# Sunshine-718/AlphaZero-AL

Hardware: AMD Instinct MI355X
Metric: self-play positions/sec (Connect4 n_playout=200, batch=8192 games/GPU, vl_batch=4) (higher is better)
Workload: dtype f32; 1 GPU; Connect4 self-play, n_playout=200, 8192 games/GPU, vl_batch=4, evaluator=cnn; c_base=1000, use_symmetry=True, lead_in_plies=12, streams_per_gpu=1, parallelism=independent game shards x1

## Files before the change

### alphazero-al_amd/csrc/nn_conv.hip

```cpp
#include <cstdio>
#include <cstdlib>

#include "az_nn.h"
#include "nn_common.h"

namespace {

constexpr int CELLS = 42, COLS = 7;
constexpr int PCOLS = 8, PCELLS = 72;
constexpr int TS = 4;
constexpr int COUT = 64;
constexpr int CELLB = 128;

template <int N>
__device__ __forceinline__ void stage_sample(const void *base, uint32_t voff, uint32_t lds_off, uint64_t last_mask)
{
    uint32_t keep;
    uint64_t ex;
    if constexpr (N == 6)
        asm volatile("s_mov_b32 %0, m0\n\ts_mov_b32 m0, %4\n\ts_nop 2\n\t"
                     "global_load_lds_dwordx4 %2, %3\n\t"
                     "global_load_lds_dwordx4 %2, %3 offset:1024\n\t"
                     "global_load_lds_dwordx4 %2, %3 offset:2048\n\t"
                     "global_load_lds_dwordx4 %2, %3 offset:3072\n\t"
                     "s_mov_b32 m0, %6\n\ts_nop 0\n\t"
                     "global_load_lds_dwordx4 %5, %3\n\t"
                     "s_and_saveexec_b64 %1, %7\n\t"
                     "global_load_lds_dwordx4 %5, %3 offset:1024\n\t"
                     "s_mov_b64 exec, %1\n\ts_mov_b32 m0, %0"
                     : "=&s"(keep), "=&s"(ex)
                     : "v"(voff), "s"(base), "s"(lds_off), "v"(voff + 4096), "s"(lds_off + 4096), "s"(last_mask)
                     : "memory", "scc");
    else
        asm volatile("s_mov_b32 %0, m0\n\ts_mov_b32 m0, %4\n\ts_nop 2\n\t"
                     "global_load_lds_dwordx4 %2, %3\n\t"
                     "global_load_lds_dwordx4 %2, %3 offset:1024\n\t"
                     "s_and_saveexec_b64 %1, %5\n\t"
                     "global_load_lds_dwordx4 %2, %3 offset:2048\n\t"
                     "s_mov_b64 exec, %1\n\ts_mov_b32 m0, %0"
                     : "=&s"(keep), "=&s"(ex)
                     : "v"(voff), "s"(base), "s"(lds_off), "s"(last_mask)
                     : "memory", "scc");
}
__device__ __forceinline__ uint32_t lds_addr(const void *p)
{
    return static_cast<uint32_t>(reinterpret_cast<uintptr_t>((__attribute__((address_space(3))) const void *)p));
}
__device__ __forceinline__ void lds_barrier()
{
    asm volatile("s_waitcnt lgkmcnt(0)" ::: "memory");
    __builtin_amdgcn_s_barrier();
    asm volatile("" ::: "memory");
}

__device__ unsigned long long g_prof[2048 * 8];

struct EmbedIn {
    const float    *features;
    const uint16_t *emb_own, *emb_opp;
    const uint16_t *pos;
    const int32_t  *gather;
    const uint64_t *bb_p1, *bb_p2;
    const int32_t  *turn, *sym;
};

struct StemIn {
    const uint64_t *bb_p1, *bb_p2;
    const int32_t  *turn, *sym;
    const int32_t  *gather;
    const uint16_t *wfrag;
    const float    *pmap;
};
constexpr int PROWS = 48, PROW = 68;
constexpr int PMAPB = PROWS * PROW * 4, FRAGB = 2 * 4 * 64 * 16;

template <int CIN, bool NORM, bool RESID, bool EMBED = false>
__global__ void __launch_bounds__(256, 2) k_conv_block(const uint16_t *x, const uint16_t *w, const uint16_t *bias,
                                                       const uint16_t *gamma, const uint16_t *beta, uint16_t *y,
                                                       int64_t B, float eps, int dbg, const int64_t *batch_dev, EmbedIn em)
{
    constexpr bool STEM = false;
    const StemIn st{};
#include "nn_conv_body.h"
}

__global__ void __launch_bounds__(256, 2) k_stem_conv_block(StemIn st, const uint16_t *w, const uint16_t *bias,
                                                            const uint16_t *gamma, const uint16_t *beta, uint16_t *y,
                                                            int64_t B, float eps, int dbg, const int64_t *batch_dev)
{
    constexpr int CIN = 64;
    constexpr bool NORM = true, RESID = true, EMBED = false, STEM = true;
    const uint16_t *x = nullptr;
    const EmbedIn em{};
#include "nn_conv_body.h"
}

int g_dbg = 0;

int prepare(DeviceSetup &setup, const void *kern, size_t smem, int c_in, int64_t B, unsigned &grid, int &dbg)
{
    if (setup.cus({kern}, static_cast<int>(smem), [&] {
            if (getenv("AZ_NN_VERBOSE") != nullptr) {
                int per_cu = 0;
                (void)hipOccupancyMaxActiveBlocksPerMultiprocessor(&per_cu, kern, 256, smem);
                if (c_in != 0)
                    fprintf(stderr, "[az_nn] conv block C_in=%d: %zu B LDS, %d workgroups per CU\n", c_in, smem, per_cu);
                else
                    fprintf(stderr, "[az_nn] stem + conv block: %zu B LDS, %d workgroups per CU\n", smem, per_cu);
            }
        }) == 0)
        return 2;
    static const int prio = [] { const char *e = getenv("AZ_NN_CONV_PRIO"); const int v = e ? atoi(e) : 1; return v < 0 || v > 3 ? 1 : v; }();
    const int64_t ntiles = (B + TS - 1) / TS;
    static const int64_t max_grid = getenv("AZ_NN_CONV_GRID") ? atoll(getenv("AZ_NN_CONV_GRID")) : 512;
    grid = static_cast<unsigned>(ntiles < max_grid ? ntiles : max_grid);
    dbg = (g_dbg & 255) | (((g_dbg >> 5) & 3) ? 0 : (prio << 5));
    return 0;
}

template <int CIN, bool NORM, bool RESID, bool EMBED = false>
int launch(const void *x, const void *w, const void *bias, const void *gamma, const void *beta, void *y, int64_t B,
           float eps, const int64_t *batch_dev, hipStream_t s, EmbedIn em = EmbedIn{})
{
    constexpr size_t smem = static_cast<size_t>(TS) * PCELLS * CELLB + 2 * static_cast<size_t>(TS) * CELLS * CIN * 2 +
                            (RESID ? 0 : static_cast<size_t>(TS) * CELLS * COUT * 2) + 2 * CIN * sizeof(float) + 512;
    auto kern = k_conv_block<CIN, NORM, RESID, EMBED>;
    static DeviceSetup setup;
    unsigned grid;
    int dbg;
    if (prepare(setup, reinterpret_cast<const void *>(kern), smem, CIN, B, grid, dbg) != 0) return 2;
    hipLaunchKernelGGL(kern, dim3(grid), dim3(256), smem, s, static_cast<const uint16_t *>(x),
                       static_cast<const uint16_t *>(w), static_cast<const uint16_t *>(bias),
                       static_cast<const uint16_t *>(gamma), static_cast<const uint16_t *>(beta),
                       static_cast<uint16_t *>(y), B, eps, dbg, batch_dev, em);
    return 0;
}

int launch_stem(const StemIn &st, const void *w, const void *bias, const void *gamma, const void *beta, void *y, int64_t B,
                float eps, const int64_t *batch_dev, hipStream_t s)
{
    constexpr size_t smem = static_cast<size_t>(TS) * PCELLS * CELLB + static_cast<size_t>(TS) * CELLS * 64 * 2 +
                            2 * 64 * sizeof(float) + 512 + PMAPB + FRAGB;
    static_assert(2 * smem <= 160 * 1024, "two workgroups per CU");
    static DeviceSetup setup;
    unsigned grid;
    int dbg;
    if (prepare(setup, reinterpret_cast<const void *>(k_stem_conv_block), smem, 0, B, grid, dbg) != 0) return 2;
    hipLaunchKernelGGL(k_stem_conv_block, dim3(grid), dim3(256), smem, s, st, static_cast<const uint16_t *>(w),
                       static_cast<const uint16_t *>(bias), static_cast<const uint16_t *>(gamma),
                       static_cast<const uint16_t *>(beta), static_cast<uint16_t *>(y), B, eps, dbg, batch_dev);
    return 0;
}

}

extern "C" {

int az_nn_debug(int flags) { g_dbg = flags; return 0; }
int az_nn_debug_flags(void) { return g_dbg; }

int az_nn_conv_profile(unsigned long long *out, int n)
{
    if (n > 2048 * 8) n = 2048 * 8;
    return hipMemcpyFromSymbol(out, HIP_SYMBOL(g_prof), sizeof(unsigned long long) * n) == hipSuccess ? 0 : 2;
}

int az_nn_conv_block(const void *x, int c_in, const void *weight_ohwi, const void *bias, const void *gamma,
                     const void *beta, int residual, void *y, int64_t batch, float eps, const int64_t *batch_dev,
                     void *stream)
{
    if (batch <= 0) return 1;
    hipStream_t s = static_cast<hipStream_t>(stream);
    const bool norm = gamma != nullptr && beta != nullptr;
    if (c_in == 64 && norm && residual) return launch<64, true, true>(x, weight_ohwi, bias, gamma, beta, y, batch, eps, batch_dev, s);
    if (c_in == 64 && norm && !residual) return launch<64, true, false>(x, weight_ohwi, bias, gamma, beta, y, batch, eps, batch_dev, s);
    if (c_in == 32 && !norm && !residual) return launch<32, false, false>(x, weight_ohwi, bias, gamma, beta, y, batch, eps, batch_dev, s);
    return 1;
}

int az_nn_stem_conv_block_positions(const az_nn_positions *positions, const void *w_frag, const float *pmap,
                                    const void *weight_ohwi, const void *bias, const void *gamma, const void *beta, void *y,
                                    int64_t batch, float eps, const int32_t *gather, const int64_t *batch_dev, void *stream)
{
    if (batch <= 0 || positions == nullptr || !positions->bb_p1 || !positions->bb_p2 || !positions->turn || !positions->sym ||
        w_frag == nullptr || pmap == nullptr || weight_ohwi == nullptr || bias == nullptr || gamma == nullptr || beta == nullptr ||
        y == nullptr)
        return 1;
    const StemIn st{positions->bb_p1, positions->bb_p2, positions->turn, positions->sym, gather,
                    static_cast<const uint16_t *>(w_frag), pmap};
    return launch_stem(st, weight_ohwi, bias, gamma, beta, y, batch, eps, batch_dev, static_cast<hipStream_t>(stream));
}

int az_nn_stem_embed(const float *features, const void *emb_own, const void *emb_opp, const void *pos,
                     const void *weight_ohwi, const void *bias, void *y, int64_t batch, const int32_t *gather,
                     const int64_t *batch_dev, void *stream)
{
    if (batch <= 0 || features == nullptr) return 1;
    EmbedIn em{features, static_cast<const uint16_t *>(emb_own), static_cast<const uint16_t *>(emb_opp),
               static_cast<const uint16_t *>(pos), gather, nullptr, nullptr, nullptr, nullptr};
    return launch<32, false, false, true>(nullptr, weight_ohwi, bias, nullptr, nullptr, y, batch, 0.0f, batch_dev,
                                          static_cast<hipStream_t>(stream), em);
}

int az_nn_stem_embed_positions(const az_nn_positions *positions, const void *emb_own, const void *emb_opp, const void *pos,
                               const void *weight_ohwi, const void *bias, void *y, int64_t batch, const int32_t *gather,
                               const int64_t *batch_dev, void *stream)
{
    if (batch <= 0 || positions == nullptr || !positions->bb_p1 || !positions->bb_p2 || !positions->turn || !positions->sym) return 1;
    EmbedIn em{nullptr, static_cast<const uint16_t *>(emb_own), static_cast<const uint16_t *>(emb_opp),
               static_cast<const uint16_t *>(pos), gather, positions->bb_p1, positions->bb_p2, positions->turn, positions->sym};
    return launch<32, false, false, true>(nullptr, weight_ohwi, bias, nullptr, nullptr, y, batch, 0.0f, batch_dev,
                                          static_cast<hipStream_t>(stream), em);
}

}
```

### alphazero-al_amd/csrc/nn_conv_body.h

```cpp
    static_assert(!EMBED || (CIN == 32 && !NORM && !RESID), "the embedding is fused into the stem only");
    static_assert(!STEM || (CIN == 64 && NORM && RESID && !EMBED), "the folded stem is fused into the first residual block only");
    constexpr int NRAW = STEM ? 1 : 2;
    const int64_t rows_total = B;
    if (batch_dev != nullptr && *batch_dev < B) B = *batch_dev;
    constexpr int K = 9 * CIN;
    constexpr int KSTEPS = K / 32;
    constexpr int KPT = CIN / 32;
    constexpr int VPC = CIN / 8;
    constexpr int VPS = CELLS * VPC;
    constexpr int PER = (VPS + 63) / 64;
    constexpr int SB = VPS * 16;
    constexpr int OVPS = CELLS * COUT / 8;
    constexpr int OPER = (OVPS + 63) / 64;
    constexpr int OSB = OVPS * 16;
    constexpr int LASTN = VPS - 64 * (PER - 1), OLASTN = OVPS - 64 * (OPER - 1);
    static_assert(LASTN > 0 && LASTN < 64 && OLASTN > 0 && OLASTN < 64 && (PER == 6 || PER == 3), "stage_sample's two forms");

    extern __shared__ __align__(16) uint8_t smem[];
    uint8_t *img = smem;
    uint8_t *rawb = smem + TS * PCELLS * CELLB;
    uint8_t *outs = rawb + NRAW * TS * SB;
    float *s_gam = reinterpret_cast<float *>(outs + (RESID ? 0 : TS * OSB)), *s_bet = s_gam + CIN;
    uint8_t *dump = reinterpret_cast<uint8_t *>(s_gam + 2 * CIN);
    uint8_t *s_pm = dump + 512, *s_fr = s_pm + PMAPB;

    const int tid = threadIdx.x;
    const int lane = tid & 63;
    const int wave = __builtin_amdgcn_readfirstlane(tid >> 6);
    const int mh = wave & 1, th = wave >> 1;
    const int l15 = lane & 15, l4 = lane >> 4;

    bf16x8 aw[2][KSTEPS];
    float bia[2][4];
#pragma unroll
    for (int mt = 0; mt < 2; ++mt) {
        const int o = mh * 32 + (l15 >> 2) * 8 + mt * 4 + (l15 & 3);
#pragma unroll
        for (int s = 0; s < KSTEPS; ++s)
            aw[mt][s] = *reinterpret_cast<const bf16x8 *>(w + static_cast<size_t>(o) * K + s * 32 + l4 * 8);
#pragma unroll
        for (int r = 0; r < 4; ++r)
            bia[mt][r] = __uint_as_float(static_cast<uint32_t>(bias[mh * 32 + l4 * 8 + mt * 4 + r]) << 16);
    }
    if (NORM && tid < CIN) {
        s_gam[tid] = __uint_as_float(static_cast<uint32_t>(gamma[tid]) << 16);
        s_bet[tid] = __uint_as_float(static_cast<uint32_t>(beta[tid]) << 16);
    }
    {
        V8 z; z.w[0] = z.w[1] = z.w[2] = z.w[3] = 0;
        constexpr int NV = (TS * PCELLS * CELLB + NRAW * TS * SB) / 16;
        for (int i = tid; i < NV; i += 256) reinterpret_cast<V8 *>(smem)[i] = z;
    }
    if (STEM) {
        for (int i = tid; i < PMAPB / 16; i += 256) reinterpret_cast<V8 *>(s_pm)[i] = reinterpret_cast<const V8 *>(st.pmap)[i];
        for (int i = tid; i < FRAGB / 16; i += 256) reinterpret_cast<V8 *>(s_fr)[i] = reinterpret_cast<const V8 *>(st.wfrag)[i];
    }
    __syncthreads();

    auto swz_in = [](int cell) { return VPC == 8 ? (cell & 7) : 0; };
    auto tok_off = [](uint32_t l, int vpc) { return vpc == 8 ? ((l >> 3) << 7) | (((l & 7) ^ ((l >> 3) & 7)) << 4) : l << 4; };
    const uint32_t raw_lds = lds_addr(rawb);
    if (EMBED) {
        for (int i = tid; i < CELLS * CIN / 8; i += 256)
            reinterpret_cast<V8 *>(rawb)[i] = reinterpret_cast<const V8 *>(em.pos)[i];
        __syncthreads();
    }
    auto stage_tile = [&](int64_t tile, int buf, uint32_t lane) {
        const int64_t b = tile * TS + wave;
        if (EMBED || STEM || b >= B) return;
        stage_sample<PER>(x + b * (CELLS * CIN), tok_off(lane, VPC), raw_lds + (buf * TS + wave) * SB, (1ull << LASTN) - 1);
    };

    const int64_t ntiles = (B + TS - 1) / TS;
    float pl_own[PER], pl_opp[PER];
    auto load_planes = [&](int64_t tile, uint32_t lane) {
        const int64_t b = tile * TS + wave;
        const bool live = b < B;
        int64_t row = !live ? 0 : (em.gather != nullptr ? em.gather[b] : b);
        if (row < 0 || row >= rows_total) row = 0;
        if (em.features != nullptr) {
            const float *fs = em.features + row * (3 * CELLS);
#pragma unroll
            for (int i = 0; i < PER; ++i) {
                const uint32_t s = lane + 64 * i;
                const bool ok = live && s < VPS;
                pl_own[i] = ok ? fs[s / VPC] : 0.0f;
                pl_opp[i] = ok ? fs[CELLS + s / VPC] : 0.0f;
            }
        } else {
            const bool p1 = em.turn[row] > 0, mir = em.sym[row] != 0;
            const uint64_t own = p1 ? em.bb_p1[row] : em.bb_p2[row], opp = p1 ? em.bb_p2[row] : em.bb_p1[row];
#pragma unroll
            for (int i = 0; i < PER; ++i) {
                const uint32_t s = lane + 64 * i;
                const bool ok = live && s < VPS;
                const int cell = ok ? s / VPC : 0;
                const int r = cell / COLS, c = cell - r * COLS;
                const int bit = (mir ? COLS - 1 - c : c) * 7 + (5 - r);
                pl_own[i] = (ok && ((own >> bit) & 1ull)) ? 1.0f : 0.0f;
                pl_opp[i] = (ok && ((opp >> bit) & 1ull)) ? 1.0f : 0.0f;
            }
        }
    };
    auto request_row = [&](int64_t tile) {
        const int64_t b = tile * TS + wave;
        int32_t r = 0;
        if (tile < ntiles && b < B && st.gather != nullptr) r = st.gather[b];
        return r;
    };
// ... 322 lines not shown
```

### alphazero-al_amd/csrc/nn_model.hip

```cpp
#include <hip/hip_runtime.h>

#include <cstdint>
#include <cstdlib>
#include <cstring>
#include <mutex>
#include <new>
#include <vector>

#include "az_nn.h"
#include "board_sym.h"

struct az_nn_model {
    int kind = AZ_NN_KIND_CONNECT4_CNN;
    bool attn_heads_fused = true;
    bool stem_fused = true;
    uint64_t hash_salt = 0;
    az_nn_model_weights w{};
    az_nn_othello_weights ow{};
};

namespace {
constexpr int64_t kTokenBytes = 42 * 64 * 2;
constexpr uint64_t kOtTok = 64 * 32 * 2, kOtMap10 = 100 * 256 * 2, kOtMap8 = 64 * 256 * 2, kOtNeck = 64 * 8 * 2;

constexpr int kKinds = 4;
struct Profile {
    std::mutex mu;
    bool on = false;
    int stride = 1;
    int64_t seen = 0;
    std::vector<hipEvent_t> start[kKinds], stop[kKinds];
    size_t used[kKinds] = {0, 0, 0, 0};
} g_prof;
constexpr size_t kProfileMax = 4096;

__device__ __forceinline__ uint64_t position_hash(uint64_t bb0, uint64_t bb1, bool p1_to_move)
{
    uint64_t x = bb0 * 0x9E3779B97F4A7C15ull;
    x ^= (bb1 + 0x7F4A7C159E3779B9ull) * 0xBF58476D1CE4E5B9ull;
    x += p1_to_move ? 0x94D049BB133111EBull : 0x2545F4914F6CDD1Dull;
    x ^= x >> 30; x *= 0xBF58476D1CE4E5B9ull;
    x ^= x >> 27; x *= 0x94D049BB133111EBull;
    x ^= x >> 31;
    return x;
}

template <bool OTHELLO>
__global__ void __launch_bounds__(256) k_hash_eval(const float *features, const uint8_t *mask, float *probs, float *wdl,
                                                   float *ml, int64_t batch, const int32_t *rows, const int64_t *n_rows, uint64_t salt)
{
    constexpr int CELLS = OTHELLO ? 64 : 42, A = OTHELLO ? 65 : 7;
    const int lane = threadIdx.x & 63;
    const int64_t b = static_cast<int64_t>(blockIdx.x) * (blockDim.x >> 6) + (threadIdx.x >> 6);
    int64_t n = batch;
    if (n_rows != nullptr && *n_rows < n) n = *n_rows;
    if (b >= n) return;
    int64_t row = rows != nullptr ? rows[b] : b;
    if (row < 0 || row >= batch) return;
    const float *f = features + row * 3 * CELLS;
    const bool in = lane < CELLS;
    const float own = in ? f[lane] : 0.0f, opp = in ? f[CELLS + lane] : 0.0f;
    const bool p1 = f[2 * CELLS] > 0.0f;
    const bool is_p1 = in && ((p1 && own != 0.0f) || (!p1 && opp != 0.0f));
    const bool is_p2 = in && ((p1 && opp != 0.0f) || (!p1 && own != 0.0f));
    uint64_t bb0 = 0, bb1 = 0;
    if (OTHELLO) {
        bb0 = __ballot(is_p1); bb1 = __ballot(is_p2);
    } else {
        const uint64_t m1 = __ballot(is_p1), m2 = __ballot(is_p2);
        for (int c = 0; c < 42; ++c) {
            const int bt = (c % 7) * 7 + (5 - c / 7);
            bb0 |= ((m1 >> c) & 1ull) << bt;
            bb1 |= ((m2 >> c) & 1ull) << bt;
        }
    }
    const uint64_t h = position_hash(bb0 ^ salt, bb1, p1);
    const uint8_t *mk = mask != nullptr ? mask + row * A : nullptr;
    if (!OTHELLO) {
        if (lane < 7) {
            const float p = static_cast<float>(1 + ((h >> (4 * lane)) & 15)) / 16.0f;
            probs[row * 7 + lane] = (mk == nullptr || mk[lane]) ? p : 0.0f;
        }
    } else {
        for (int a = lane; a < 65; a += 64) {
            const int k = a >> 4, j = a & 15;
            uint64_t hk = h + 0x9E3779B97F4A7C15ull * static_cast<uint64_t>(k + 1);
            hk ^= hk >> 29; hk *= 0xBF58476D1CE4E5B9ull; hk ^= hk >> 32;
            const float p = static_cast<float>(1 + ((hk >> (4 * j)) & 15)) / 16.0f;
            probs[row * 65 + a] = (mk == nullptr || mk[a]) ? p : 0.0f;
        }
    }
    if (lane < 3) {
        const uint64_t w0 = 1 + ((h >> 28) & 31), w1 = 1 + ((h >> 33) & 31), w2 = 1 + ((h >> 38) & 31);
        const float tot = static_cast<float>(w0 + w1 + w2);
        const uint64_t mine = lane == 0 ? w0 : (lane == 1 ? w1 : w2);
        wdl[row * 3 + lane] = static_cast<float>(mine) / tot;
    }
    if (lane == 3) {
// ... 51 lines not shown
{
    if (positions == nullptr || mask == nullptr) return 1;
    if (scratch == nullptr || scratch_bytes < az_nn_model_scratch_bytes(m, batch)) return 1;
    const az_nn_othello_weights &o = m->ow;
    char *base = static_cast<char *>(scratch);
    char *tok = base; base += batch * kOtTok;
    char *map[3];
    for (auto &p : map) { p = base; base += batch * kOtMap10; }
    char *pa = base; base += batch * kOtMap8;
    char *pb = base; base += batch * kOtMap8;
    char *neck = base;
    auto conv = [&](int i, const void *x, const void *res, void *y) {
        const az_nn_othello_conv_layer &l = o.conv[i];
        return az_nn_othello_conv(x, l.w_packed, l.pre_scale, l.pre_shift, l.post_scale, l.post_shift, l.residual ? res : nullptr,
                                  y, batch, l.c_in, l.h_in, l.pad, 1, n_rows, stream);
    };
    int rc = az_nn_othello_embed(positions, mask, o.embed_table, tok, batch, rows, n_rows, stream);
    int cur = 0;
    if (rc == 0) rc = conv(0, tok, nullptr, map[cur]);
    for (int i = 1; rc == 0 && i + 1 < o.n_body; i += 2) {
        const int y1 = (cur + 1) % 3, y2 = (cur + 2) % 3;
        rc = conv(i, map[cur], nullptr, map[y1]);
        if (rc == 0) rc = conv(i + 1, map[y1], map[cur], map[y2]);
        cur = y2;
    }
    const int hid = (cur + 1) % 3;
    if (rc == 0) rc = conv(o.n_body - 1, map[cur], nullptr, map[hid]);
    if (rc == 0) rc = conv(o.n_body, map[hid], nullptr, pa);
    if (rc == 0) rc = conv(o.n_body + 1, pa, nullptr, pb);
    if (rc == 0) rc = az_nn_othello_conv_narrow(map[hid], o.dual_w16, o.dual_scale16, o.dual_shift16, neck, batch, n_rows, stream);
    if (rc == 0) rc = az_nn_othello_heads(pb, neck, &o.heads, probs, wdl, moves_left, batch, rows, n_rows, stream);
    return rc;
}

int forward_hash(const az_nn_model *m, const float *features, const az_nn_positions *positions, const uint8_t *mask,
                 float *probs, float *wdl, float *moves_left, int64_t batch, const int32_t *rows, const int64_t *n_rows,
                 void *stream)
{
    if (positions != nullptr) {
        const dim3 grid(static_cast<unsigned>((batch + 255) / 256)), block(256);
        if (m->kind == AZ_NN_KIND_HASH_OTHELLO)
            hipLaunchKernelGGL(k_hash_eval_positions<true>, grid, block, 0, static_cast<hipStream_t>(stream), *positions, mask, probs,
                               wdl, moves_left, batch, rows, n_rows, m->hash_salt);
        else
            hipLaunchKernelGGL(k_hash_eval_positions<false>, grid, block, 0, static_cast<hipStream_t>(stream), *positions, mask, probs,
                               wdl, moves_left, batch, rows, n_rows, m->hash_salt);
        return 0;
    }
    const dim3 grid(static_cast<unsigned>((batch + 3) / 4)), block(256);
    if (m->kind == AZ_NN_KIND_HASH_OTHELLO)
        hipLaunchKernelGGL(k_hash_eval<true>, grid, block, 0, static_cast<hipStream_t>(stream), features, mask, probs, wdl,
                           moves_left, batch, rows, n_rows, m->hash_salt);
    else
        hipLaunchKernelGGL(k_hash_eval<false>, grid, block, 0, static_cast<hipStream_t>(stream), features, mask, probs, wdl,
                           moves_left, batch, rows, n_rows, m->hash_salt);
    return 0;
}

int forward_connect4(const az_nn_model *m, const float *features, const az_nn_positions *positions, const uint8_t *mask,
                     float *probs, float *wdl, float *moves_left, int64_t batch, const int32_t *rows, const int64_t *n_rows,
                     void *scratch, uint64_t scratch_bytes, void *stream)
{
    if (scratch == nullptr || scratch_bytes < az_nn_model_scratch_bytes(m, batch)) return 1;
    const az_nn_model_weights &w = m->w;
    char *a = static_cast<char *>(scratch);
    char *b = a + batch * kTokenBytes;
    hipStream_t hs = static_cast<hipStream_t>(stream);
    bool timed = false;
    int slot[kKinds] = {-1, -1, -1, -1};
    if (g_prof.on) {
        std::lock_guard<std::mutex> lk(g_prof.mu);
        hipStreamCaptureStatus cs = hipStreamCaptureStatusNone;
        const bool capturing = hipStreamIsCapturing(hs, &cs) == hipSuccess && cs != hipStreamCaptureStatusNone;
        if (g_prof.on && !capturing && (g_prof.seen++ % g_prof.stride) == 0) {
            timed = true;
            for (int kd = 0; kd < kKinds; ++kd)
                if (g_prof.used[kd] < g_prof.start[kd].size()) slot[kd] = static_cast<int>(g_prof.used[kd]++);
        }
    }
    auto begin = [&](int kd) { if (timed && slot[kd] >= 0) (void)hipEventRecord(g_prof.start[kd][slot[kd]], hs); };
    auto end = [&](int kd) { if (timed && slot[kd] >= 0) (void)hipEventRecord(g_prof.stop[kd][slot[kd]], hs); };
    int rc;
    int first = 0;
    if (m->stem_fused && !timed && positions != nullptr && w.stem_frag != nullptr && w.stem_pmap != nullptr && w.n_blocks >= 1) {
        rc = az_nn_stem_conv_block_positions(positions, w.stem_frag, w.stem_pmap, w.block_w[0], w.block_b[0], w.block_gamma[0],
                                             w.block_beta[0], a, batch, w.eps, rows, n_rows, stream);
        first = 1;
    } else {
        begin(AZ_NN_PROFILE_STEM);
        if (w.stem_frag != nullptr && w.stem_pmap != nullptr)
            rc = positions != nullptr
                ? az_nn_stem_folded_positions(positions, w.stem_frag, w.stem_pmap, a, batch, rows, n_rows, stream)
                : az_nn_stem_folded(features, w.stem_frag, w.stem_pmap, a, batch, rows, n_rows, stream);
        else
            rc = positions != nullptr
                ? az_nn_stem_embed_positions(positions, w.emb_own, w.emb_opp, w.pos, w.stem_w, w.stem_b, a, batch, rows, n_rows, stream)
                : az_nn_stem_embed(features, w.emb_own, w.emb_opp, w.pos, w.stem_w, w.stem_b, a, batch, rows, n_rows, stream);
        end(AZ_NN_PROFILE_STEM);
    }
    for (int i = first; rc == 0 && i < w.n_blocks; ++i) {
        if (i == 0) begin(AZ_NN_PROFILE_CONV);
        rc = az_nn_conv_block(a, 64, w.block_w[i], w.block_b[i], w.block_gamma[i], w.block_beta[i], 1, b, batch,
                              w.eps, n_rows, stream);
        if (i == 0) end(AZ_NN_PROFILE_CONV);
        char *t = a; a = b; b = t;
    }
    if (rc == 0 && m->attn_heads_fused && !timed)
        return az_nn_attn_heads(a, w.pre_w, w.qkvg_w, w.qn_w, w.kn_w, w.o_w, &w.heads, mask, probs, wdl, moves_left, batch,
                                w.eps, rows, n_rows, stream);
    if (rc == 0) {
        begin(AZ_NN_PROFILE_ATTN);
        rc = az_nn_attn_block(a, w.pre_w, w.qkvg_w, w.qn_w, w.kn_w, w.o_w, b, batch, w.eps, n_rows, stream);
        end(AZ_NN_PROFILE_ATTN);
        char *t = a; a = b; b = t;
    }
    if (rc == 0) {
        begin(AZ_NN_PROFILE_HEADS);
        rc = az_nn_heads(a, &w.heads, mask, probs, wdl, moves_left, batch, w.eps, rows, n_rows, stream);
        end(AZ_NN_PROFILE_HEADS);
    }
    return rc;
}

int forward(const az_nn_model *m, const float *features, const az_nn_positions *positions, const uint8_t *mask, float *probs,
            float *wdl, float *moves_left, int64_t batch, const int32_t *rows, const int64_t *n_rows, void *scratch,
            uint64_t scratch_bytes, void *stream)
{
    if (m == nullptr || probs == nullptr || wdl == nullptr || moves_left == nullptr) return 1;
    if (batch <= 0) return batch == 0 ? 0 : 1;
    if ((rows == nullptr) != (n_rows == nullptr)) return 1;
    if (m->kind == AZ_NN_KIND_OTHELLO_CNN)
        return forward_othello(m, positions, mask, probs, wdl, moves_left, batch, rows, n_rows, scratch, scratch_bytes, stream);
    if (m->kind != AZ_NN_KIND_CONNECT4_CNN)
        return forward_hash(m, features, positions, mask, probs, wdl, moves_left, batch, rows, n_rows, stream);
    return forward_connect4(m, features, positions, mask, probs, wdl, moves_left, batch, rows, n_rows, scratch, scratch_bytes, stream);
}

}

extern "C" {

int az_nn_model_create(const az_nn_model_weights *w, az_nn_model **out)
{
    if (w == nullptr || out == nullptr) return 1;
    if (w->n_blocks < 0 || w->n_blocks > AZ_NN_MAX_BLOCKS) return 1;
    if ((w->stem_frag == nullptr) != (w->stem_pmap == nullptr)) return 1;
    const void *need[] = {w->emb_own, w->emb_opp, w->pos, w->stem_w, w->stem_b, w->pre_w, w->qkvg_w,
                          w->qn_w, w->kn_w, w->o_w, w->heads.p_norm, w->heads.d_val_w};
    for (const void *p : need)
        if (p == nullptr) return 1;
    for (int i = 0; i < w->n_blocks; ++i)
        if (!w->block_w[i] || !w->block_b[i] || !w->block_gamma[i] || !w->block_beta[i]) return 1;
    auto *m = new (std::nothrow) az_nn_model();
    if (m == nullptr) return 1;
    m->w = *w;
    const char *fused = getenv("AZ_ATTN_HEADS_FUSED");
    m->attn_heads_fused = fused == nullptr || strcmp(fused, "0") != 0;
    const char *stem = getenv("AZ_STEM_FUSED");
    m->stem_fused = stem == nullptr || strcmp(stem, "0") != 0;
    *out = m;
    return 0;
}

int az_nn_model_create_hash_salted(int game, uint64_t salt, az_nn_model **out)
{
    if (out == nullptr || (game != 0 && game != 1)) return 1;
    auto *m = new (std::nothrow) az_nn_model();
    if (m == nullptr) return 1;
    m->kind = game == 0 ? AZ_NN_KIND_HASH_CONNECT4 : AZ_NN_KIND_HASH_OTHELLO;
    m->hash_salt = salt;
    *out = m;
    return 0;
}

int az_nn_model_create_hash(int game, az_nn_model **out) { return az_nn_model_create_hash_salted(game, 0, out); }

int az_nn_model_create_othello(const az_nn_othello_weights *w, az_nn_model **out)
{
    if (w == nullptr || out == nullptr || w->embed_table == nullptr) return 1;
    if (w->n_body < 2 || w->n_body % 2 != 0 || w->n_convs != w->n_body + 2 || w->n_convs > AZ_NN_OTHELLO_MAX_CONVS) return 1;
    for (int i = 0; i < w->n_convs; ++i)
        if (!w->conv[i].w_packed || !w->conv[i].post_scale || !w->conv[i].post_shift) return 1;
    if (!w->dual_w16 || !w->dual_scale16 || !w->dual_shift16 || !w->heads.board_w || !w->heads.a_fc_wt) return 1;
    auto *m = new (std::nothrow) az_nn_model();
    if (m == nullptr) return 1;
    m->kind = AZ_NN_KIND_OTHELLO_CNN;
    m->ow = *w;
    *out = m;
    return 0;
}

void az_nn_model_destroy(az_nn_model *m) { delete m; }

int az_nn_model_kind(const az_nn_model *m) { return m ? m->kind : -1; }

uint64_t az_nn_model_scratch_bytes(const az_nn_model *m, int64_t batch)
{
    if (m != nullptr && m->kind == AZ_NN_KIND_OTHELLO_CNN)
        return batch > 0 ? static_cast<uint64_t>(batch) * (kOtTok + 3 * kOtMap10 + 2 * kOtMap8 + kOtNeck) : 0;
    if (m != nullptr && m->kind != AZ_NN_KIND_CONNECT4_CNN) return 0;
    return batch > 0 ? static_cast<uint64_t>(2 * batch * kTokenBytes) : 0;
}

int az_nn_model_forward(const az_nn_model *m, const float *features, const uint8_t *mask, float *probs,
                        float *wdl, float *moves_left, int64_t batch, const int32_t *rows,
                        const int64_t *n_rows, void *scratch, uint64_t scratch_bytes, void *stream)
{
    if (features == nullptr) return 1;
    return forward(m, features, nullptr, mask, probs, wdl, moves_left, batch, rows, n_rows, scratch, scratch_bytes, stream);
}

int az_nn_model_forward_positions(const az_nn_model *m, const az_nn_positions *positions, const uint8_t *mask, float *probs,
                                  float *wdl, float *moves_left, int64_t batch, const int32_t *rows,
                                  const int64_t *n_rows, void *scratch, uint64_t scratch_bytes, void *stream)
{
    if (positions == nullptr || !positions->bb_p1 || !positions->bb_p2 || !positions->turn || !positions->sym) return 1;
    return forward(m, nullptr, positions, mask, probs, wdl, moves_left, batch, rows, n_rows, scratch, scratch_bytes, stream);
}

int az_nn_model_profile(int enable)
{
    std::lock_guard<std::mutex> lk(g_prof.mu);
    if (enable) {
        for (int kd = 0; kd < kKinds; ++kd)
            while (g_prof.start[kd].size() < kProfileMax) {
                hipEvent_t a, b;
                if (hipEventCreate(&a) != hipSuccess || hipEventCreate(&b) != hipSuccess) return 2;
                g_prof.start[kd].push_back(a); g_prof.stop[kd].push_back(b);
            }
    }
    g_prof.on = enable != 0;
    g_prof.stride = enable > 1 ? enable : 1;
    g_prof.seen = 0;
    return 0;
}

int az_nn_model_profile_read_kernels(double out_ms[4], int64_t out_launches[4])
{
    if (out_ms == nullptr || out_launches == nullptr) return 1;
    if (hipDeviceSynchronize() != hipSuccess) return 2;
    std::lock_guard<std::mutex> lk(g_prof.mu);
    for (int kd = 0; kd < kKinds; ++kd) {
// ... 26 lines not shown
```

### alphazero-al_amd/src/abi.py

```python
import ctypes as C
import os

import torch


class SearchConfig(C.Structure):
    _fields_ = [(n, C.c_float) for n in ("c_init", "c_base", "dirichlet_alpha", "noise_epsilon", "fpu_reduction", "mlh_slope",
                                         "mlh_cap", "score_utility_factor", "score_scale", "value_decay")] + \
               [("use_symmetry", C.c_uint8), ("vl_count", C.c_int32)]


class SelfPlayConfig(C.Structure):
    _fields_ = [("temperature", C.c_float), ("temp_endgame", C.c_float), ("temp_decay_moves", C.c_int32),
                ("refill", C.c_int32), ("record", C.c_int32), ("noise_steps", C.c_int32),
                ("max_finished_games", C.c_int64), ("noise_eps_init", C.c_double), ("noise_eps_min", C.c_double)]


class SelfPlayGames(C.Structure):
    _fields_ = [(n, C.c_void_p) for n in ("slot", "length", "winner", "finish_ply", "row_start", "bb_p1", "bb_p2",
                                          "turn", "prob", "wdl", "mask")]


class ReplayTensorsC(C.Structure):
    _fields_ = [(n, C.c_void_p) for n in ("state", "prob", "winner", "steps_to_end", "aux_target", "root_wdl",
# ... 149 lines not shown
    ("az_mcts_search_rollout", i32, [vp, vp, vp, i64, i32]),
    ("az_mcts_search_rollout_dev", i32, [vp, vp, vp, i64, i32]),
    ("az_mcts_get_all_counts", i32, [vp, vp]),
    ("az_mcts_get_all_root_stats", i32, [vp, vp]),
    ("az_mcts_dev_prepare", i32, [vp, i32, i64]),
    ("az_mcts_dev_prepare_stream", i32, [vp, i32, i64, vp]),
    ("az_mcts_dev_check", i32, [vp, vp]),
    ("az_mcts_dev_replay", i32, [vp, vp, i64, i64, vp]),
    ("az_mcts_dev_set_roots", i32, [vp, vp, vp, vp, vp]),
    ("az_mcts_dev_import_roots", i32, [vp, vp, vp, vp]),
    ("az_mcts_dev_select", i32, [vp, i32, i32, vp, vp, vp]),
    ("az_mcts_dev_backprop", i32, [vp, i32, i32, vp, vp, vp, vp]),
    ("az_mcts_dev_leaves", i32, [vp, i32, vp, vp, vp, vp, vp]),
    ("az_mcts_dev_leaf_syms", i32, [vp, i32, vp, vp]),
    ("az_mcts_dev_counts", i32, [vp, vp, vp]),
    ("az_mcts_dev_root_stats", i32, [vp, vp, vp]),
    ("az_mcts_dev_prune_roots", i32, [vp, vp, vp]),
    ("az_mcts_dev_reset_masked", i32, [vp, vp, vp]),
    ("az_c4_dev_step", i32, [vp, vp, vp, vp, vp, vp, i64, i32, vp]),
    ("az_game_dev_step", i32, [i32, vp, vp, vp, vp, vp, vp, vp, i64, i32, vp]),
    ("az_game_dev_valid_mask", i32, [i32, vp, vp, vp, vp, vp, i64, vp]),
    ("az_mcts_dev_set_noise_epsilons", i32, [vp, vp]),
    ("az_mcts_dev_live_leaves", i32, [vp, i32, vp, vp, vp]),
    ("az_mcts_dev_search", i32, [vp, vp, i32, i32, i32, vp]),
    ("az_mcts_dev_search_more", i32, [vp, vp, i32, i32, i32, vp]),
    ("az_mcts_dev_rollout_search", i32, [vp, i32, i32, vp]),
    ("az_selfplay_create", i32, [vp, P(SelfPlayConfig), P(vp)]),
    ("az_selfplay_destroy", None, [vp]),
    ("az_selfplay_step", i32, [vp, vp, i32, i32, i32, i32, vp]),
    ("az_selfplay_begin_ply", i32, [vp, vp]),
    ("az_selfplay_finish_ply", i32, [vp, vp]),
    ("az_selfplay_set_action_tape", i32, [vp, vp, i64]),
    ("az_selfplay_totals", i32, [vp, P(i64 * 5)]),
    ("az_selfplay_positions", i32, [vp, vp, vp, vp, vp]),
    ("az_selfplay_finished", i32, [vp, P(i64), P(i64), P(i64)]),
    ("az_selfplay_drain", i32, [vp, P(SelfPlayGames), i64, i64]),
    ("az_selfplay_export", i32, [vp, P(ReplayTensorsC), i64, i32, i64, i64, P(SelfPlayExportInfo), P(i64), vp]),
    ("az_replay_dev_store", i32, [i32, P(SelfPlayGames), vp, vp, i64, P(ReplayTensorsC), i64, i32, vp]),
    ("az_selfplay_sample", i32, [i32, vp, vp, P(SelfPlayConfig), u64, u64, vp, i64, vp]),
    ("az_selfplay_create_teams", i32, [vp, P(SelfPlayConfig), vp, P(vp)]),
    ("az_selfplay_team_sample", i32, [i32, vp, vp, P(SelfPlayConfig), i32, i32, u64, u64, vp, vp, vp, i64, vp]),
    ("az_mcts_dev_team_root_stats", i32, [i32, vp, i32, i32, vp, i64, vp]),
    ("az_match_create", i32, [vp, vp, P(MatchConfig), P(vp)]),
    ("az_match_create_teams", i32, [vp, vp, P(MatchConfig), vp, P(vp)]),
    ("az_match_destroy", None, [vp]),
    ("az_match_set_positions", i32, [vp, vp, vp, vp]),
    ("az_match_step", i32, [vp, vp, vp, i32, i32, i32, i32, vp]),
    ("az_match_step_players", i32, [vp, vp, vp, i32, i32, i32, i32, i32, i32, vp]),
    ("az_match_begin_ply", i32, [vp, vp, P(i32)]),
    ("az_match_finish_ply", i32, [vp, vp]),
    ("az_match_set_action_tape", i32, [vp, vp, i64]),
    ("az_match_remaining", i32, [vp, P(i64)]),
    ("az_match_results", i32, [vp, vp, vp, P(i64 * 4)]),
    ("az_match_moves", i32, [vp, vp]),
    ("az_match_max_plies", i32, [vp]),
    ("az_match_sample", i32, [i32, vp, f32, u64, u64, vp, i64, vp]),
    ("az_match_team_roots", i32, [i32, vp, vp, vp, i32, i32, vp, vp, vp, i64, vp]),
    ("az_match_team_sample", i32, [i32, vp, i32, i32, f32, u64, u64, vp, vp, i32, i32, vp, i64, vp]),
    ("az_game_num_augment", i32, [i32]),
    ("az_replay_dev_batch", i32, [i32, P(ReplayTensorsC), vp, vp, i64, i64, P(ReplayBatchC), vp]),
    ("az_replay_dev_sample_indices", i32, [u64, u64, i64, vp, i64, vp]),
    ("az_mcts_dev_tt_create", i32, [vp, i32]),
    ("az_mcts_dev_tt_clear", i32, [vp, vp]),
    ("az_mcts_dev_tt_lookup", i32, [vp, i32, vp, vp, vp, vp, vp, vp]),
    ("az_mcts_dev_tt_insert", i32, [vp, i32, vp, vp, vp, vp, vp, vp]),
    ("az_mcts_dev_tt_refresh", i32, [vp, vp, vp]),
    ("az_mcts_dev_tt_stats", i32, [vp, P(i64 * 4)]),
    ("az_mcts_reserve", i32, [vp, i64]),
    ("az_mcts_capacity", i64, [vp]),
    ("az_mcts_epoch", i64, [vp]),
    ("az_mcts_max_used", i32, [vp, P(i64)]),
    ("az_mcts_counters", i32, [vp, P(i64 * 8)]),
    ("az_mcts_counters_reset", i32, [vp]),
    ("az_mcts_profile", i32, [vp, i32]),
    ("az_mcts_profile_read", i32, [vp, P(C.c_double * 2), P(i64 * 2)]),
    ("az_mcts_timed_select_kernel", cstr, [vp]),
    ("az_rng_gamma_selftest", i32, [u32, f32, i32, vp]),
    ("az_nn_stem_embed", i32, [vp, vp, vp, vp, vp, vp, vp, i64, vp, vp, vp]),
    ("az_nn_stem_embed_positions", i32, [P(Positions), vp, vp, vp, vp, vp, vp, i64, vp, vp, vp]),
    ("az_nn_stem_folded", i32, [vp, vp, vp, vp, i64, vp, vp, vp]),
    ("az_nn_stem_folded_positions", i32, [P(Positions), vp, vp, vp, i64, vp, vp, vp]),
    ("az_nn_conv_block", i32, [vp, i32, vp, vp, vp, vp, i32, vp, i64, f32, vp, vp]),
    ("az_nn_stem_conv_block_positions", i32, [P(Positions), vp, vp, vp, vp, vp, vp, vp, i64, f32, vp, vp, vp]),
    ("az_nn_attn_block", i32, [vp, vp, vp, vp, vp, vp, vp, i64, f32, vp, vp]),
    ("az_nn_heads", i32, [vp, P(HeadsWeights), vp, vp, vp, vp, i64, f32, vp, vp, vp]),
    ("az_nn_attn_heads", i32, [vp, vp, vp, vp, vp, vp, P(HeadsWeights), vp, vp, vp, vp, i64, f32, vp, vp, vp]),
    ("az_nn_model_create", i32, [P(ModelWeights), P(vp)]),
    ("az_nn_model_create_hash", i32, [i32, P(vp)]),
    ("az_nn_model_create_hash_salted", i32, [i32, u64, P(vp)]),
    ("az_nn_model_kind", i32, [vp]),
    ("az_nn_model_destroy", None, [vp]),
    ("az_nn_model_scratch_bytes", u64, [vp, i64]),
    ("az_nn_model_forward", i32, [vp, vp, vp, vp, vp, vp, i64, vp, vp, vp, u64, vp]),
    ("az_nn_model_forward_positions", i32, [vp, P(Positions), vp, vp, vp, vp, i64, vp, vp, vp, u64, vp]),
    ("az_nn_model_profile", i32, [i32]),
    ("az_nn_model_profile_read", i32, [P(C.c_double), P(i64)]),
    ("az_nn_model_profile_read_kernels", i32, [P(C.c_double * 4), P(i64 * 4)]),
    ("az_nn_debug", i32, [i32]),
    ("az_nn_debug_flags", i32, []),
    ("az_nn_conv_profile", i32, [vp, i32]),
    ("az_nn_debug_col_reduce2", i32, [vp, vp, vp, vp]),
    ("az_nn_embed", i32, [vp, vp, vp, vp, vp, i64, i32, vp, vp, vp]),
    ("az_nn_heads_prep", i32, [vp, vp, vp, f32, vp, vp, i64, f32, vp]),
    ("az_nn_othello_conv", i32, [vp, vp, vp, vp, vp, vp, vp, vp, i64, i32, i32, i32, i32, vp, vp]),
    ("az_nn_othello_conv_narrow", i32, [vp, vp, vp, vp, vp, i64, vp, vp]),
    ("az_nn_othello_embed", i32, [P(Positions), vp, vp, vp, i64, vp, vp, vp]),
    ("az_nn_othello_heads", i32, [vp, vp, P(_HeadsW), vp, vp, vp, i64, vp, vp, vp]),
    ("az_nn_model_create_othello", i32, [P(_OthelloW), P(vp)]),
    ("az_train_loss_workspace_bytes", i64, [i32, i64]),
    ("az_train_dev_loss", i32, [i32, P(ReplayBatchC), P(TrainHeadsC), i64, P(TrainLossConfigC), P(TrainLossOutC), vp]),
    ("az_train_dev_loss_grad", i32, [i32, P(ReplayBatchC), P(TrainHeadsC), i64, P(TrainLossConfigC), P(TrainLossOutC), vp,
                                     P(TrainGradsC), vp]),
    ("az_opt_create", i32, [i64, vp, vp, i32, P(vp)]),
    ("az_opt_destroy", None, [vp]),
    ("az_opt_bind", i32, [vp, vp, vp, vp]),
    ("az_opt_dev_step", i32, [vp, vp, vp, vp, f32, vp, vp]),
    ("az_train_block_workspace_bytes", i64, [i64, i32]),
    ("az_train_dev_block_fwd", i32, [vp, vp, vp, i64, f32, vp, vp, vp]),
    ("az_train_dev_block_bwd", i32, [vp, vp, vp, vp, vp, i64, i32, vp, vp]),
    ("az_train_attn_workspace_bytes", i64, [i64, i32]),
    ("az_train_dev_attn_fwd", i32, [vp, vp, i32, vp, f32, i64, f32, vp, vp]),
    ("az_train_dev_attn_bwd", i32, [vp, vp, i32, vp, f32, vp, i64, f32, i32, vp, vp]),
    ("az_train_stem_workspace_bytes", i64, [i64, i32]),
    ("az_train_dev_stem_fwd", i32, [vp, vp, i64, vp, vp, i64, vp]),
    ("az_train_dev_stem_bwd", i32, [vp, vp, vp, vp, i64, i32, vp, vp]),
    ("az_train_heads_workspace_bytes", i64, [i64, i32]),
    ("az_train_dev_heads_fwd", i32, [vp, vp, vp, vp, vp, i64, f32, vp, vp, vp, vp]),
    ("az_train_dev_heads_bwd", i32, [vp, vp, vp, vp, vp, vp, vp, vp, i64, f32, i32, vp, vp]),
)

_LIB = None


def lib():
    global _LIB
    if _LIB is None:
        L = C.CDLL(os.path.join(os.path.dirname(os.path.dirname(os.path.abspath(__file__))), "lib", "libaz_mcts.so"))
        for name, restype, argtypes in PROTOTYPES:
            fn = getattr(L, name)
            fn.restype, fn.argtypes = restype, argtypes
        _LIB = L
    return _LIB


def glue():
    try:
        return lib()
    except OSError:
        return None


def check(rc):
    if rc != 0:
        raise RuntimeError(lib().az_last_error().decode())


def _stream():
    return C.c_void_p(torch.cuda.current_stream().cuda_stream)


def counters(handle):
    arr = (C.c_int64 * 8)()
    check(lib().az_mcts_counters(handle, C.byref(arr)))
    names = ("sims", "levels", "expansions", "terminal", "dup_leaves", "backup_nodes",
             "select_launches", "backprop_launches")
    return dict(zip(names, list(arr)))
# ... 1 lines not shown
```

### include/az_nn.h

```cpp
#ifndef AZ_NN_H
#define AZ_NN_H

#include <stdint.h>

#ifdef __cplusplus
extern "C" {
#endif


int az_nn_stem_embed(const float *features, const void *emb_own, const void *emb_opp, const void *pos,
                     const void *weight_ohwi, const void *bias, void *y, int64_t batch, const int32_t *gather,
                     const int64_t *batch_dev, void *stream);
typedef struct az_nn_positions {
    const uint64_t *bb_p1, *bb_p2;
    const int32_t *turn, *sym;
} az_nn_positions;
int az_nn_stem_embed_positions(const az_nn_positions *positions, const void *emb_own, const void *emb_opp, const void *pos,
                               const void *weight_ohwi, const void *bias, void *y, int64_t batch, const int32_t *gather,
                               const int64_t *batch_dev, void *stream);
int az_nn_stem_folded(const float *features, const void *w_frag, const float *pmap, void *y, int64_t batch,
                      const int32_t *gather, const int64_t *batch_dev, void *stream);
int az_nn_stem_folded_positions(const az_nn_positions *positions, const void *w_frag, const float *pmap, void *y,
                                int64_t batch, const int32_t *gather, const int64_t *batch_dev, void *stream);
int az_nn_conv_block(const void *x, int c_in, const void *weight_ohwi, const void *bias, const void *gamma,
                     const void *beta, int residual, void *y, int64_t batch, float eps, const int64_t *batch_dev,
                     void *stream);
int az_nn_stem_conv_block_positions(const az_nn_positions *positions, const void *w_frag, const float *pmap,
                                    const void *weight_ohwi, const void *bias, const void *gamma, const void *beta, void *y,
                                    int64_t batch, float eps, const int32_t *gather, const int64_t *batch_dev, void *stream);
int az_nn_attn_block(const void *x, const void *prenorm_w, const void *qkvg_w, const void *q_norm_w,
                     const void *k_norm_w, const void *o_w, void *y, int64_t batch, float eps, const int64_t *batch_dev,
                     void *stream);
typedef struct az_nn_heads_weights {
    const void *p_norm, *p_gate_w, *p_fc_w, *p_fc_b, *p_out_w;
    const void *d_pool_norm, *d_pool_w, *d_pool_b, *d_norm, *d_fc_w, *d_fc_b, *d_out_norm;
    const void *d_val_w, *d_val_b, *d_aux_w;
    float p_gate_b, p_out_b, d_aux_b, aux_scale;
} az_nn_heads_weights;
int az_nn_heads(const void *tokens, const az_nn_heads_weights *w, const uint8_t *mask, float *probs, float *wdl,
                float *moves_left, int64_t batch, float eps, const int32_t *scatter, const int64_t *batch_dev,
                void *stream);
int az_nn_attn_heads(const void *x, const void *prenorm_w, const void *qkvg_w, const void *q_norm_w, const void *k_norm_w,
                     const void *o_w, const az_nn_heads_weights *w, const uint8_t *mask, float *probs, float *wdl,
                     float *moves_left, int64_t batch, float eps, const int32_t *scatter, const int64_t *batch_dev,
                     void *stream);


#define AZ_NN_MAX_BLOCKS 8
typedef struct az_nn_model_weights {
    const void *emb_own, *emb_opp, *pos;
    const void *stem_w, *stem_b;
    int32_t n_blocks;
    const void *block_w[AZ_NN_MAX_BLOCKS], *block_b[AZ_NN_MAX_BLOCKS];
    const void *block_gamma[AZ_NN_MAX_BLOCKS], *block_beta[AZ_NN_MAX_BLOCKS];
    const void *pre_w, *qkvg_w, *qn_w, *kn_w, *o_w;
    az_nn_heads_weights heads;
    float eps;
    const void *stem_frag;
    const float *stem_pmap;
} az_nn_model_weights;
typedef struct az_nn_model az_nn_model;
int az_nn_model_create(const az_nn_model_weights *w, az_nn_model **out);
int az_nn_model_create_hash(int game, az_nn_model **out);
int az_nn_model_create_hash_salted(int game, uint64_t salt, az_nn_model **out);
#define AZ_NN_KIND_CONNECT4_CNN  0
#define AZ_NN_KIND_HASH_CONNECT4 1
#define AZ_NN_KIND_HASH_OTHELLO  2
int az_nn_model_kind(const az_nn_model *m);
void az_nn_model_destroy(az_nn_model *m);
uint64_t az_nn_model_scratch_bytes(const az_nn_model *m, int64_t batch);
int az_nn_model_forward(const az_nn_model *m, const float *features, const uint8_t *mask, float *probs,
                        float *wdl, float *moves_left, int64_t batch, const int32_t *rows,
                        const int64_t *n_rows, void *scratch, uint64_t scratch_bytes, void *stream);
int az_nn_model_forward_positions(const az_nn_model *m, const az_nn_positions *positions, const uint8_t *mask, float *probs,
                                  float *wdl, float *moves_left, int64_t batch, const int32_t *rows,
                                  const int64_t *n_rows, void *scratch, uint64_t scratch_bytes, void *stream);
int az_nn_model_profile(int enable);
int az_nn_model_profile_read(double *out_ms, int64_t *out_launches);
#define AZ_NN_PROFILE_STEM  0
#define AZ_NN_PROFILE_CONV  1
#define AZ_NN_PROFILE_ATTN  2
#define AZ_NN_PROFILE_HEADS 3
int az_nn_model_profile_read_kernels(double out_ms[4], int64_t out_launches[4]);


#define AZ_NN_DEBUG_GRID_CAP(n) (((n) & 0xfff) << 16)
int az_nn_debug(int flags);
int az_nn_debug_flags(void);
int az_nn_conv_profile(unsigned long long *out, int n);
int az_nn_debug_col_reduce2(const float *a, const float *b, float *out, void *stream);


int az_nn_embed(const float *features, const void *emb_own, const void *emb_opp, const void *pos,
                void *tokens, int64_t batch, int embed_dim, const int32_t *gather, const int64_t *batch_dev,
                void *stream);
int az_nn_heads_prep(const void *tokens, const void *p_norm_w, const void *p_gate_w, float p_gate_b,
                     void *col, void *mean, int64_t batch, float eps, void *stream);


int az_nn_othello_conv(const void *x, const void *w_packed, const float *pre_scale, const float *pre_shift,
                       const float *post_scale, const float *post_shift, const void *residual, void *y,
                       int64_t batch, int c_in, int h_in, int pad, int apply_silu, const int64_t *batch_dev, void *stream);

int az_nn_othello_conv_narrow(const void *x, const void *w_packed16, const float *post_scale16,
                              const float *post_shift16, void *y, int64_t batch, const int64_t *batch_dev, void *stream);

typedef struct az_nn_othello_heads_weights {
    const void  *board_w;
    const float *pass_norm_w, *pass_fc_w;
    const float *v_conv_w;
    const float *v_bn_s, *v_bn_b;
    const float *v_fc_w, *v_fc_b;
// ... 33 lines not shown
```

Measured before the change: 302,300 positions/s.

## Fuse stem and all residual conv blocks into one persistent chained kernel

Adds a k_conv_chain kernel that runs the fused stem conv block and then loops over the remaining residual conv blocks inside one launch, ping-ponging outputs between two buffers. Between layers it waits on outstanding memory ops, issues an agent-scope acquire fence and a workgroup barrier. This removes per-layer kernel launch overhead and inter-kernel gaps. Correctness relies on each workgroup reading only tiles it wrote itself, since there is no grid-wide barrier, and all layers must use the larger shared-memory size of the stem and block variants. It is on by default and can be disabled with AZ_CONV_CHAIN=0.

Result: faster. 310,300 positions/s (median of 6 runs) (+2.6%).

```diff
diff --git a/alphazero-al_amd/csrc/nn_conv.hip b/alphazero-al_amd/csrc/nn_conv.hip
--- a/alphazero-al_amd/csrc/nn_conv.hip
+++ b/alphazero-al_amd/csrc/nn_conv.hip
@@ -79,7 +79,7 @@
                                                        const uint16_t *gamma, const uint16_t *beta, uint16_t *y,
                                                        int64_t B, float eps, int dbg, const int64_t *batch_dev, EmbedIn em)
 {
-    constexpr bool STEM = false;
+    constexpr bool STEM = false, CHAINED = false;
     const StemIn st{};
 #include "nn_conv_body.h"
 }
@@ -89,10 +89,48 @@
                                                             int64_t B, float eps, int dbg, const int64_t *batch_dev)
 {
     constexpr int CIN = 64;
-    constexpr bool NORM = true, RESID = true, EMBED = false, STEM = true;
+    constexpr bool NORM = true, RESID = true, EMBED = false, STEM = true, CHAINED = false;
     const uint16_t *x = nullptr;
     const EmbedIn em{};
 #include "nn_conv_body.h"
+}
+
+struct ChainIn {
+    const uint16_t *w[AZ_NN_MAX_BLOCKS], *bias[AZ_NN_MAX_BLOCKS], *gamma[AZ_NN_MAX_BLOCKS], *beta[AZ_NN_MAX_BLOCKS];
+    uint16_t *y[AZ_NN_MAX_BLOCKS];
+    int n;
+};
+
+__device__ __forceinline__ void layer_switch()
+{
+    asm volatile("s_waitcnt vmcnt(0)" ::: "memory");
+    __builtin_amdgcn_fence(__ATOMIC_ACQUIRE, "agent");
+    __syncthreads();
+}
+
+__global__ void __launch_bounds__(256, 2) k_conv_chain(StemIn st_in, ChainIn ch, int64_t B, float eps, int dbg, const int64_t *batch_dev_in)
+{
+    constexpr int CIN = 64;
+    constexpr bool NORM = true, RESID = true, EMBED = false;
+    const EmbedIn em{};
+    {
+        constexpr bool STEM = true, CHAINED = false;
+        const StemIn &st = st_in;
+        const uint16_t *x = nullptr, *w = ch.w[0], *bias = ch.bias[0], *gamma = ch.gamma[0], *beta = ch.beta[0];
+        uint16_t *y = ch.y[0];
+        const int64_t *batch_dev = batch_dev_in;
+#include "nn_conv_body.h"
+    }
+#pragma unroll 1
+    for (int layer = 1; layer < ch.n; ++layer) {
+        layer_switch();
+        constexpr bool STEM = false, CHAINED = true;
+        const StemIn st{};
+        const uint16_t *x = ch.y[layer - 1], *w = ch.w[layer], *bias = ch.bias[layer], *gamma = ch.gamma[layer], *beta = ch.beta[layer];
+        uint16_t *y = ch.y[layer];
+        const int64_t *batch_dev = nullptr;
+#include "nn_conv_body.h"
+    }
 }
 
 int g_dbg = 0;
@@ -103,7 +141,9 @@
             if (getenv("AZ_NN_VERBOSE") != nullptr) {
                 int per_cu = 0;
                 (void)hipOccupancyMaxActiveBlocksPerMultiprocessor(&per_cu, kern, 256, smem);
-                if (c_in != 0)
+                if (c_in < 0)
+                    fprintf(stderr, "[az_nn] stem + conv chain: %zu B LDS, %d workgroups per CU\n", smem, per_cu);
+                else if (c_in != 0)
                     fprintf(stderr, "[az_nn] conv block C_in=%d: %zu B LDS, %d workgroups per CU\n", c_in, smem, per_cu);
                 else
                     fprintf(stderr, "[az_nn] stem + conv block: %zu B LDS, %d workgroups per CU\n", smem, per_cu);
@@ -152,6 +192,22 @@
     return 0;
 }
 
+int launch_chain(const StemIn &st, const ChainIn &ch, int64_t B, float eps, const int64_t *batch_dev, hipStream_t s)
+{
+    constexpr size_t smem_block = static_cast<size_t>(TS) * PCELLS * CELLB + 2 * static_cast<size_t>(TS) * CELLS * 64 * 2 +
+                                  2 * 64 * sizeof(float) + 512;
+    constexpr size_t smem_stem = static_cast<size_t>(TS) * PCELLS * CELLB + static_cast<size_t>(TS) * CELLS * 64 * 2 +
+                                 2 * 64 * sizeof(float) + 512 + PMAPB + FRAGB;
+    constexpr size_t smem = smem_block > smem_stem ? smem_block : smem_stem;
+    static_assert(smem == 80896 && 2 * smem <= 160 * 1024, "two workgroups per CU");
+    static DeviceSetup setup;
+    unsigned grid;
+    int dbg;
+    if (prepare(setup, reinterpret_cast<const void *>(k_conv_chain), smem, -1, B, grid, dbg) != 0) return 2;
+    hipLaunchKernelGGL(k_conv_chain, dim3(grid), dim3(256), smem, s, st, ch, B, eps, dbg, batch_dev);
+    return 0;
+}
+
 }
 
 extern "C" {
@@ -191,6 +247,30 @@
     return launch_stem(st, weight_ohwi, bias, gamma, beta, y, batch, eps, batch_dev, static_cast<hipStream_t>(stream));
 }
 
+int az_nn_stem_conv_chain_positions(const az_nn_positions *positions, const void *w_frag, const float *pmap, int n_blocks,
+                                    const void *const *weight_ohwi, const void *const *bias, const void *const *gamma,
+                                    const void *const *beta, void *y_even, void *y_odd, int64_t batch, float eps,
+                                    const int32_t *gather, const int64_t *batch_dev, void *stream)
+{
+    if (batch <= 0 || positions == nullptr || !positions->bb_p1 || !positions->bb_p2 || !positions->turn || !positions->sym ||
+        w_frag == nullptr || pmap == nullptr || n_blocks < 1 || n_blocks > AZ_NN_MAX_BLOCKS || weight_ohwi == nullptr ||
+        bias == nullptr || gamma == nullptr || beta == nullptr || y_even == nullptr || y_odd == nullptr || y_even == y_odd)
+        return 1;
+    ChainIn ch{};
+    for (int i = 0; i < n_blocks; ++i) {
+        if (!weight_ohwi[i] || !bias[i] || !gamma[i] || !beta[i]) return 1;
+        ch.w[i] = static_cast<const uint16_t *>(weight_ohwi[i]);
+        ch.bias[i] = static_cast<const uint16_t *>(bias[i]);
+        ch.gamma[i] = static_cast<const uint16_t *>(gamma[i]);
+        ch.beta[i] = static_cast<const uint16_t *>(beta[i]);
+        ch.y[i] = static_cast<uint16_t *>((i & 1) ? y_odd : y_even);
+    }
+    ch.n = n_blocks;
+    const StemIn st{positions->bb_p1, positions->bb_p2, positions->turn, positions->sym, gather,
+                    static_cast<const uint16_t *>(w_frag), pmap};
+    return launch_chain(st, ch, batch, eps, batch_dev, static_cast<hipStream_t>(stream));
+}
+
 int az_nn_stem_embed(const float *features, const void *emb_own, const void *emb_opp, const void *pos,
                      const void *weight_ohwi, const void *bias, void *y, int64_t batch, const int32_t *gather,
                      const int64_t *batch_dev, void *stream)
diff --git a/alphazero-al_amd/csrc/nn_conv_body.h b/alphazero-al_amd/csrc/nn_conv_body.h
--- a/alphazero-al_amd/csrc/nn_conv_body.h
+++ b/alphazero-al_amd/csrc/nn_conv_body.h
@@ -24,7 +24,8 @@
     uint8_t *dump = reinterpret_cast<uint8_t *>(s_gam + 2 * CIN);
     uint8_t *s_pm = dump + 512, *s_fr = s_pm + PMAPB;
 
-    const int tid = threadIdx.x;
+    int tid = threadIdx.x;
+    if (CHAINED) asm volatile("" : "+v"(tid));
     const int lane = tid & 63;
     const int wave = __builtin_amdgcn_readfirstlane(tid >> 6);
     const int mh = wave & 1, th = wave >> 1;
diff --git a/alphazero-al_amd/csrc/nn_model.hip b/alphazero-al_amd/csrc/nn_model.hip
--- a/alphazero-al_amd/csrc/nn_model.hip
+++ b/alphazero-al_amd/csrc/nn_model.hip
@@ -14,6 +14,7 @@
     int kind = AZ_NN_KIND_CONNECT4_CNN;
     bool attn_heads_fused = true;
     bool stem_fused = true;
+    bool conv_chain = true;
     uint64_t hash_salt = 0;
     az_nn_model_weights w{};
     az_nn_othello_weights ow{};
@@ -231,7 +232,13 @@
     auto end = [&](int kd) { if (timed && slot[kd] >= 0) (void)hipEventRecord(g_prof.stop[kd][slot[kd]], hs); };
     int rc;
     int first = 0;
-    if (m->stem_fused && !timed && positions != nullptr && w.stem_frag != nullptr && w.stem_pmap != nullptr && w.n_blocks >= 1) {
+    if (m->stem_fused && m->conv_chain && !timed && positions != nullptr && w.stem_frag != nullptr && w.stem_pmap != nullptr &&
+        w.n_blocks >= 2) {
+        rc = az_nn_stem_conv_chain_positions(positions, w.stem_frag, w.stem_pmap, w.n_blocks, w.block_w, w.block_b, w.block_gamma,
+                                             w.block_beta, a, b, batch, w.eps, rows, n_rows, stream);
+        first = w.n_blocks;
+        if ((w.n_blocks & 1) == 0) { char *t = a; a = b; b = t; }
+    } else if (m->stem_fused && !timed && positions != nullptr && w.stem_frag != nullptr && w.stem_pmap != nullptr && w.n_blocks >= 1) {
         rc = az_nn_stem_conv_block_positions(positions, w.stem_frag, w.stem_pmap, w.block_w[0], w.block_b[0], w.block_gamma[0],
                                              w.block_beta[0], a, batch, w.eps, rows, n_rows, stream);
         first = 1;
@@ -307,6 +314,8 @@
     m->attn_heads_fused = fused == nullptr || strcmp(fused, "0") != 0;
     const char *stem = getenv("AZ_STEM_FUSED");
     m->stem_fused = stem == nullptr || strcmp(stem, "0") != 0;
+    const char *chain = getenv("AZ_CONV_CHAIN");
+    m->conv_chain = chain == nullptr || strcmp(chain, "0") != 0;
     *out = m;
     return 0;
 }
diff --git a/alphazero-al_amd/src/abi.py b/alphazero-al_amd/src/abi.py
--- a/alphazero-al_amd/src/abi.py
+++ b/alphazero-al_amd/src/abi.py
@@ -255,6 +255,7 @@
     ("az_nn_stem_folded_positions", i32, [P(Positions), vp, vp, vp, i64, vp, vp, vp]),
     ("az_nn_conv_block", i32, [vp, i32, vp, vp, vp, vp, i32, vp, i64, f32, vp, vp]),
     ("az_nn_stem_conv_block_positions", i32, [P(Positions), vp, vp, vp, vp, vp, vp, vp, i64, f32, vp, vp, vp]),
+    ("az_nn_stem_conv_chain_positions", i32, [P(Positions), vp, vp, i32, vp, vp, vp, vp, vp, vp, i64, f32, vp, vp, vp]),
     ("az_nn_attn_block", i32, [vp, vp, vp, vp, vp, vp, vp, i64, f32, vp, vp]),
     ("az_nn_heads", i32, [vp, P(HeadsWeights), vp, vp, vp, vp, i64, f32, vp, vp, vp]),
     ("az_nn_attn_heads", i32, [vp, vp, vp, vp, vp, vp, P(HeadsWeights), vp, vp, vp, vp, i64, f32, vp, vp, vp]),
diff --git a/include/az_nn.h b/include/az_nn.h
--- a/include/az_nn.h
+++ b/include/az_nn.h
@@ -28,6 +28,10 @@
 int az_nn_stem_conv_block_positions(const az_nn_positions *positions, const void *w_frag, const float *pmap,
                                     const void *weight_ohwi, const void *bias, const void *gamma, const void *beta, void *y,
                                     int64_t batch, float eps, const int32_t *gather, const int64_t *batch_dev, void *stream);
+int az_nn_stem_conv_chain_positions(const az_nn_positions *positions, const void *w_frag, const float *pmap, int n_blocks,
+                                    const void *const *weight_ohwi, const void *const *bias, const void *const *gamma,
+                                    const void *const *beta, void *y_even, void *y_odd, int64_t batch, float eps,
+                                    const int32_t *gather, const int64_t *batch_dev, void *stream);
 int az_nn_attn_block(const void *x, const void *prenorm_w, const void *qkvg_w, const void *q_norm_w,
                      const void *k_norm_w, const void *o_w, void *y, int64_t batch, float eps, const int64_t *batch_dev,
                      void *stream);
```
